# DRL-Navigation/DDRL4NAV

Measured on AMD Instinct MI355X. Metric: env-steps/sec (whole node) + PPO update ms, Pong 256 envs at 1/2/4/8 GPUs, higher is better.
Workload: dtype f32 (f16x3 MFMA planes, fp32 accumulate)

## Files before the change

ddrl4nav_amd/csrc/conv2.hip:

```cpp
#include "engine2.h"

namespace ddrl {


using bf8 = __attribute__((ext_vector_type(8))) __bf16;
using u4v = __attribute__((ext_vector_type(4))) unsigned;
using bf4 = __attribute__((ext_vector_type(4))) __bf16;

#ifndef DDRL_F1_KO
#define DDRL_F1_KO 0
#endif
#ifndef DDRL_F1_LDS_PAD
#define DDRL_F1_LDS_PAD 0
#endif
#ifndef DDRL_F1_PITCH
#define DDRL_F1_PITCH 168
#endif
template <int NE>
struct Fwd1B {
  static constexpr int ROWS = 32 * NE, A_BYTES = 4 * NPL * 2 * ROWS * 16, PITCH = DDRL_F1_PITCH, IMG_BYTES = 64 * PITCH;
  static constexpr int STAGE_BYTES = A_BYTES + IMG_BYTES, AQ = A_BYTES / 16, NAJ = AQ / 256;
  static constexpr size_t LDS_BYTES = 2 * STAGE_BYTES + DDRL_F1_LDS_PAD;
};

// ... 663 lines not shown
  {
    ProfRange pr(c.prof, acting ? "ConvFwd1.act" : "ConvFwd1", st);
    if (c.L->NE == 2) {
      launch_fwd1_planes<2>(c, acting, st);
    } else {
      launch_fwd1_planes<1>(c, acting, st);
    }
  }
  {
    ProfRange pr(c.prof, acting ? "ConvFwd2.act" : "ConvFwd2", st);
    launch_fwd2_planes(c, acting, st);
  }
  {
    ProfRange pr(c.prof, acting ? "ConvFwd3.act" : "ConvFwd3", st);
    launch_fwd3_planes(c, acting, st);
  }
}

#ifndef DDRL_D3B_THREADS
#define DDRL_D3B_THREADS 256
#endif
#ifndef DDRL_D3B_TN
#define DDRL_D3B_TN 2
#endif
struct Dgrad3B {
  static constexpr int THREADS = DDRL_D3B_THREADS, TN = DDRL_D3B_TN, SPT = ((THREADS / 64) * 32 * TN) / 81;
  static constexpr int KOC = 16, NKB = 64 / KOC, PIXB = 2 * KOC;
  static constexpr int IMG_PLANE = SPT * 121 * PIXB;
  static constexpr int W_OFF = NPL * IMG_PLANE, W_BYTES = 9 * NPL * 64 * 32;
  static constexpr int NIU = SPT * 49, NIJ = (NIU + THREADS - 1) / THREADS;
  static constexpr int NWQ = W_BYTES / 16, NWJ = (NWQ + THREADS - 1) / THREADS;
  static constexpr size_t LDS_BYTES = W_OFF + W_BYTES;
};

__global__ __launch_bounds__(Dgrad3B::THREADS) __attribute__((amdgpu_waves_per_eu(2, 2))) void conv_dgrad3_planes_kernel(
    const float* __restrict__ dz3, int64_t dz_es, const unsigned short* __restrict__ wd3b, float* __restrict__ amax, const unsigned* __restrict__ m2,
    float* __restrict__ out, int64_t out_es, int n) {
  using K = Dgrad3B;
  extern __shared__ __attribute__((aligned(16))) char ldsd3[];
  const int tid = threadIdx.x, lane = tid & 63, wc = tid >> 6, l31 = lane & 31, hi = lane >> 5;
  const int e = blockIdx.z, b0 = blockIdx.x * K::SPT;
  const float sa = plane_scale(amax[amax_idx(AMAX_DZ3, e)]), inv = 1.0f / (sa * plane_scale(amax[amax_idx(AMAX_W3, e)]));
  for (int i = tid; i < K::W_OFF / 16; i += K::THREADS) *(f4*)(ldsd3 + i * 16) = zero4();
  const float* isrc[K::NIJ];
  int idst[K::NIJ];
#pragma unroll
  for (int j = 0; j < K::NIJ; ++j) {
    const int u = min(tid + K::THREADS * j, K::NIU - 1);
    const int s = u / 49, px = u % 49;
    isrc[j] = dz3 + e * dz_es + (int64_t)min(b0 + s, n - 1) * FLAT + px;
    idst[j] = (s * 121 + (px / 7 + 2) * 11 + px % 7 + 2) * K::PIXB;
  }
  const unsigned short* wsrc = wd3b + (int64_t)e * (K::NKB * 9 * NPL * 64 * 16) + tid * 8;
  int aA[2], bB[K::TN];
#pragma unroll
  for (int i = 0; i < 2; ++i) aA[i] = K::W_OFF + (i * 32 + l31) * 32 + hi * 16;
#pragma unroll
  for (int j = 0; j < K::TN; ++j) {
    int c = wc * (32 * K::TN) + j * 32 + l31;
    if (c >= K::SPT * 81) c = 0;
    const int s = c / 81, pix = c % 81;
    bB[j] = (s * 121 + (pix / 9 + 2) * 11 + pix % 9 + 2) * K::PIXB + hi * 16;
  }
  float ir[K::NIJ][K::KOC];
  f4 wr[K::NWJ];
  auto fetch = [&](int kb) {
#pragma unroll
    for (int j = 0; j < K::NIJ; ++j)
#pragma unroll
      for (int c = 0; c < K::KOC; ++c) ir[j][c] = isrc[j][(kb * K::KOC + c) * 49];
#pragma unroll
    for (int j = 0; j < K::NWJ; ++j)
      if (j + 1 < K::NWJ || tid + K::THREADS * j < K::NWQ) wr[j] = *(const f4*)(wsrc + kb * (9 * NPL * 1024) + j * (K::THREADS * 8));
  };
  auto commit = [&]() {
#pragma unroll
    for (int j = 0; j < K::NIJ; ++j) {
      if (j + 1 < K::NIJ || tid + K::THREADS * j < K::NIU) {
        unsigned pl[K::KOC / 2][NPL];
#pragma unroll
        for (int c = 0; c < K::KOC / 2; ++c) split_planes(ir[j][2 * c], ir[j][2 * c + 1], sa, pl[c]);
        char* d = ldsd3 + idst[j];
#pragma unroll
        for (int p = 0; p < NPL; ++p) {
          *(u4v*)(d + p * K::IMG_PLANE) = (u4v){pl[0][p], pl[1][p], pl[2][p], pl[3][p]};
          *(u4v*)(d + p * K::IMG_PLANE + 16) = (u4v){pl[4][p], pl[5][p], pl[6][p], pl[7][p]};
        }
      }
    }
#pragma unroll
    for (int j = 0; j < K::NWJ; ++j)
      if (j + 1 < K::NWJ || tid + K::THREADS * j < K::NWQ) *(f4*)(ldsd3 + K::W_OFF + (tid + K::THREADS * j) * 16) = wr[j];
  };
  f32x16 acc[2][K::TN];
#pragma unroll
  for (int i = 0; i < 2; ++i)
#pragma unroll
    for (int j = 0; j < K::TN; ++j)
#pragma unroll
      for (int r = 0; r < 16; ++r) acc[i][j][r] = 0.0f;
  fetch(0);
  __syncthreads();
  commit();
  fetch(1);
  __syncthreads();
  for (int kb = 0; kb < K::NKB; ++kb) {
#pragma unroll
    for (int t = 0; t < 9; ++t) {
      constexpr int ROW11 = 11;
      const int toff = ((t / 3) * ROW11 + t % 3) * K::PIXB;
      frag8 af[NPL][2], bfr[NPL][K::TN];
#pragma unroll
      for (int p = 0; p < NPL; ++p) {
#pragma unroll
        for (int i = 0; i < 2; ++i) af[p][i] = *(const frag8*)(ldsd3 + aA[i] + (t * NPL + p) * 2048);
#pragma unroll
        for (int j = 0; j < K::TN; ++j) bfr[p][j] = *(const frag8*)(ldsd3 + bB[j] - toff + p * K::IMG_PLANE);
      }
      DDRL_PLANE_PRODUCTS;
#pragma unroll
      for (int m = 0; m < NPROD; ++m)
#pragma unroll
        for (int i = 0; i < 2; ++i)
#pragma unroll
          for (int j = 0; j < K::TN; ++j) acc[i][j] = mfma_planes(af[PA[m]][i], bfr[PB[m]][j], acc[i][j]);
    }
    __syncthreads();
    if (kb + 1 < K::NKB) {
      commit();
      if (kb + 2 < K::NKB) fetch(kb + 2);
    }
    __syncthreads();
  }
  float big = 0.0f;
#pragma unroll
  for (int j = 0; j < K::TN; ++j) {
    const int c = wc * (32 * K::TN) + j * 32 + l31;
    const int s = c / 81, pix = c % 81;
    if (c >= K::SPT * 81 || b0 + s >= n) continue;
    const int64_t off = (int64_t)(b0 + s) * 5184 + pix + hi * (4 * 81);
    float* op = out + e * out_es + off;
    const unsigned mw = m2[(e * (out_es / 5184) + b0 + s) * 162 + pix * 2 + hi];
#pragma unroll
    for (int i = 0; i < 2; ++i)
#pragma unroll
      for (int r = 0; r < 16; ++r) {
        const float g = leaky_bit(mw, 16 * i + 15 - r, acc[i][j][r] * inv);
        op[(i * 32 + acc_row(r, 0)) * 81] = g;
        big = fmaxf(big, fabsf(g));
      }
  }
  amax_update(big, amax + amax_idx(AMAX_DZ2, e));
}
static void launch_dgrad3_planes(const EncCall& c, hipStream_t st) {
  using K = Dgrad3B;
  const Workspace& w = *c.ws;
  static bool configured = false;
  if (!configured) {
    (void)hipFuncSetAttribute((const void*)conv_dgrad3_planes_kernel, hipFuncAttributeMaxDynamicSharedMemorySize, (int)K::LDS_BYTES);
    configured = true;
  }
  hipLaunchKernelGGL(conv_dgrad3_planes_kernel, dim3((unsigned)((c.n + K::SPT - 1) / K::SPT), 1, (unsigned)c.L->NE), dim3(K::THREADS), K::LDS_BYTES, st,
                     w.dz3, c.max_batch * FLAT, w.wd3b, w.amax, w.m2, w.dz2, c.max_batch * 5184, c.n);
}

void launch_conv_dgrad3_2(const EncCall& c, hipStream_t st) {
  ProfRange pr(c.prof, "ConvDgrad3", st);
  launch_dgrad3_planes(c, st);
}

#ifndef DDRL_D2_KO
#define DDRL_D2_KO 0
#endif
struct Dgrad2Both {
  static constexpr int SPT = 5, THREADS = 512, TN = 2;
  static constexpr int IMG_PLANE = SPT * 121 * 16;
  static constexpr int W_HALF = 2 * NPL * 64 * 32;
  static constexpr int W_OFF = NPL * IMG_PLANE, W_BYTES = 2 * W_HALF;
  static constexpr int NIU = SPT * 81;
  static constexpr int NWQ = W_BYTES / 16, NWJ = NWQ / THREADS;
  static constexpr size_t LDS_BYTES = W_OFF + W_BYTES;
};

__global__ __launch_bounds__(512) __attribute__((amdgpu_waves_per_eu(2, 2))) void conv_dgrad2_both_kernel(
    const float* __restrict__ dz2, int64_t dz_es, const unsigned short* __restrict__ wd2b, float* __restrict__ amax, float* __restrict__ out,
    int64_t out_es, int n) {
  using K = Dgrad2Both;
  extern __shared__ __attribute__((aligned(16))) char ldsd2[];
  const int tid = threadIdx.x, lane = tid & 63, wc = tid >> 6, l31 = lane & 31, hi = lane >> 5;
  const int e = blockIdx.y, b0 = blockIdx.x * K::SPT;
  const float sa = plane_scale(amax[amax_idx(AMAX_DZ2, e)]), inv = 1.0f / (sa * plane_scale(amax[amax_idx(AMAX_W2, e)]));
  for (int i = tid; i < K::W_OFF / 16; i += K::THREADS) *(f4*)(ldsd2 + i * 16) = zero4();
  const int u = min(tid, K::NIU - 1);
  const float* isrc = dz2 + e * dz_es + (int64_t)min(b0 + u / 81, n - 1) * 5184 + u % 81;
  const int idst = ((u / 81) * 121 + ((u % 81) / 9 + 1) * 11 + (u % 81) % 9 + 1) * 16;
  const unsigned short* wsrc[K::NWJ];
#pragma unroll
  for (int j = 0; j < K::NWJ; ++j) {
    const int q = tid + K::THREADS * j, par = q / (K::W_HALF / 16), qh = q % (K::W_HALF / 16);
    wsrc[j] = wd2b + (int64_t)(e * 2 + par) * (8 * 2 * NPL * 64 * 16) + qh * 8;
  }
  int aA[4], bB[K::TN];
#pragma unroll
  for (int i = 0; i < 4; ++i) aA[i] = K::W_OFF + (i >> 1) * K::W_HALF + ((i & 1) * 32 + l31) * 32 + hi * 16;
#pragma unroll
  for (int j = 0; j < K::TN; ++j) {
    int c = wc * (32 * K::TN) + j * 32 + l31;
    if (c >= K::SPT * 100) c = 0;
    const int s = c / 100, pq = c % 100;
    bB[j] = (s * 121 + (pq / 10 + 1) * 11 + (pq % 10 + 1) - hi) * 16;
  }
  float ir[8];
  f4 wr[K::NWJ];
  auto fetch = [&](int kb) {
#pragma unroll
    for (int c = 0; c < 8; ++c) ir[c] = isrc[(kb * 8 + c) * 81];
#pragma unroll
    for (int j = 0; j < K::NWJ; ++j) wr[j] = *(const f4*)(wsrc[j] + kb * (2 * NPL * 1024));
  };
  auto commit = [&]() {
    if (tid < K::NIU) {
      unsigned pl[4][NPL];
#pragma unroll
      for (int c = 0; c < 4; ++c) split_planes(ir[2 * c], ir[2 * c + 1], sa, pl[c]);
      char* d = ldsd2 + idst;
#pragma unroll
      for (int p = 0; p < NPL; ++p) *(u4v*)(d + p * K::IMG_PLANE) = (u4v){pl[0][p], pl[1][p], pl[2][p], pl[3][p]};
    }
#pragma unroll
    for (int j = 0; j < K::NWJ; ++j) *(f4*)(ldsd2 + K::W_OFF + (tid + K::THREADS * j) * 16) = wr[j];
  };
  f32x16 acc[4][K::TN];
#pragma unroll
  for (int i = 0; i < 4; ++i)
#pragma unroll
    for (int j = 0; j < K::TN; ++j)
#pragma unroll
      for (int r = 0; r < 16; ++r) acc[i][j][r] = 0.0f;
  constexpr int NKB = 8;
  fetch(0);
  __syncthreads();
  commit();
  fetch(1);
  __syncthreads();
  for (int kb = 0; kb < NKB; ++kb) {
#pragma unroll
    for (int kg = 0; kg < 2; ++kg) {
      frag8 af[NPL][4], bfr[NPL][K::TN];
#pragma unroll
      for (int p = 0; p < NPL; ++p) {
#pragma unroll
        for (int i = 0; i < 4; ++i) af[p][i] = *(const frag8*)(ldsd2 + aA[i] + (kg * NPL + p) * 2048);
#pragma unroll
        for (int j = 0; j < K::TN; ++j) bfr[p][j] = *(const frag8*)(ldsd2 + bB[j] + p * K::IMG_PLANE - kg * (11 * 16));
      }
      DDRL_PLANE_PRODUCTS;
#pragma unroll
      for (int t = 0; t < NPROD; ++t)
#pragma unroll
        for (int i = 0; i < 4; ++i)
#pragma unroll
          for (int j = 0; j < K::TN; ++j) acc[i][j] = mfma_planes(af[PA[t]][i], bfr[PB[t]][j], acc[i][j]);
    }
    __syncthreads();
    if (kb + 1 < NKB) {
      commit();
      if (kb + 2 < NKB) fetch(kb + 2);
    }
    __syncthreads();
  }
  float big = 0.0f;
#pragma unroll
  for (int j = 0; j < K::TN; ++j) {
    const int c = wc * (32 * K::TN) + j * 32 + l31;
    const int s = c / 100, pq = c % 100;
    if (c >= K::SPT * 100 || b0 + s >= n) continue;
#pragma unroll
    for (int a = 0; a < 2; ++a) {
      float* base = out + e * out_es + (int64_t)(b0 + s) * 12800 + (2 * (pq / 10) + a) * 20 + 2 * (pq % 10);
#pragma unroll
      for (int r = 0; r < 16; ++r) {
        const float g0 = acc[2 * a][j][r] * inv, g1 = acc[2 * a + 1][j][r] * inv;
        *(float2*)(base + acc_row(r, hi) * 400) = make_float2(g0, g1);
        big = fmaxf(big, fmaxf(fabsf(g0), fabsf(g1)));
      }
    }
  }
  amax_update(big, amax + amax_idx(AMAX_DZ1, e));
}

void launch_conv_dgrad2_2(const EncCall& c, hipStream_t st) {
  const Workspace& w = *c.ws;
  ProfRange pr(c.prof, "ConvDgrad2", st);
  static bool configured = false;
  if (!configured) {
    (void)hipFuncSetAttribute((const void*)conv_dgrad2_both_kernel, hipFuncAttributeMaxDynamicSharedMemorySize, (int)Dgrad2Both::LDS_BYTES);
    configured = true;
  }
  hipLaunchKernelGGL(conv_dgrad2_both_kernel, dim3((unsigned)((c.n + Dgrad2Both::SPT - 1) / Dgrad2Both::SPT), (unsigned)c.L->NE, 1),
                     dim3(Dgrad2Both::THREADS), Dgrad2Both::LDS_BYTES, st, w.dz2, c.max_batch * 5184, w.wd2b, w.amax, w.dz1, c.max_batch * 12800, c.n);
}

}
```

ddrl4nav_amd/csrc/fc2.hip:

```cpp
#include "engine2.h"

namespace ddrl {

using bf8f = __attribute__((ext_vector_type(8))) __bf16;

#ifndef DDRL_FC_SWZ
#define DDRL_FC_SWZ 1
#endif

struct FcFwdB {
  static constexpr int PITCH = 80, PLANE = 128 * PITCH, B_OFF = NPL * PLANE, LDS_BYTES = 2 * NPL * PLANE;
};

template <bool SPLIT>
__global__ __launch_bounds__(256) void fc_fwd_planes_kernel(const float* __restrict__ a3, int64_t a3_es, const unsigned short* __restrict__ wlb,
                                                            const float* __restrict__ amax, const float* __restrict__ params, int64_t bias_off0,
                                                            int64_t bias_off1, float* __restrict__ h, int64_t h_es, int n, int ne, int nsplit,
                                                            float* __restrict__ part, const float* __restrict__ smax, int smax_es) {
  using K = FcFwdB;
  extern __shared__ __attribute__((aligned(16))) char ldsf[];
  const int tid = threadIdx.x, lane = tid & 63, wave = tid >> 6, l31 = lane & 31, hi = lane >> 5;
  const int wr = wave >> 1, wc = wave & 1;
  int bx = blockIdx.x, by = blockIdx.y, bz = blockIdx.z;
  if (!SPLIT && DDRL_FC_SWZ != 0 && (gridDim.y & 7) == 0) {
// ... 152 lines not shown
    static bool configured = false;
    if (!configured) {
      (void)hipFuncSetAttribute((const void*)fc_fwd_planes_kernel<false>, hipFuncAttributeMaxDynamicSharedMemorySize, (int)FcFwdB::LDS_BYTES);
      (void)hipFuncSetAttribute((const void*)fc_fwd_planes_kernel<true>, hipFuncAttributeMaxDynamicSharedMemorySize, (int)FcFwdB::LDS_BYTES);
      configured = true;
    }
    const dim3 grid(FEAT / 128, (c.n + 127) / 128, c.L->NE * nsplit);
    if (nsplit > 1)
      hipLaunchKernelGGL(fc_fwd_planes_kernel<true>, grid, dim3(256), FcFwdB::LDS_BYTES, st, w.a3, MB * FLAT, w.wlb, w.amax, c.params,
                         c.L->enc_base[0] + c.L->enc.lb, c.L->enc_base[c.L->NE - 1] + c.L->enc.lb, w.h, MB * FEAT, c.n, c.L->NE, nsplit, w.wpart,
                         per_sample_max ? w.actmax : (const float*)nullptr, DDRL_ACT_FUSED_MAX);
    else
      hipLaunchKernelGGL(fc_fwd_planes_kernel<false>, grid, dim3(256), FcFwdB::LDS_BYTES, st, w.a3, MB * FLAT, w.wlb, w.amax, c.params,
                         c.L->enc_base[0] + c.L->enc.lb, c.L->enc_base[c.L->NE - 1] + c.L->enc.lb, w.h, MB * FEAT, c.n, c.L->NE, 1, w.wpart,
                         (const float*)nullptr, 0);
  }
}

#ifndef DDRL_FCD_KBK
#define DDRL_FCD_KBK 32
#endif
#ifndef DDRL_FCD_WPE
#define DDRL_FCD_WPE 2
#endif
struct FcDgradB {
  static constexpr int KBK = DDRL_FCD_KBK, WPE = DDRL_FCD_WPE, PITCH = 2 * KBK + 16, PLANE = 128 * PITCH, B_OFF = NPL * PLANE, LDS_BYTES = 2 * NPL * PLANE;
  static constexpr int NAQ = KBK / 4, ARJ = 128 * NAQ / 256, AROWS = 256 / NAQ;
  static constexpr int NWF = KBK / 8, WJ = 128 * NWF / 256, WCOLS = 256 / NWF;
};
__global__ __launch_bounds__(256) __attribute__((amdgpu_waves_per_eu(FcDgradB::WPE, FcDgradB::WPE))) void fc_dgrad_planes_kernel(const float* __restrict__ dh, int64_t dh_es, const unsigned short* __restrict__ wdlb,
                                                              float* __restrict__ amax, const unsigned* __restrict__ m3, float* __restrict__ dz3, int64_t a3_es, int n) {
  using K = FcDgradB;
  extern __shared__ __attribute__((aligned(16))) char ldsg[];
  const int tid = threadIdx.x, lane = tid & 63, wave = tid >> 6, l31 = lane & 31, hi = lane >> 5;
  const int wr = wave >> 1, wc = wave & 1;
  int bx = blockIdx.x, by = blockIdx.y;
  if (DDRL_FC_SWZ != 0 && (gridDim.y & 7) == 0) {
    const int lin = bx + 25 * by, xcd = lin & 7, q = lin >> 3;
    if ((gridDim.y & 63) != 0) {
      bx = q % 25, by = (q / 25) * 8 + xcd;
    } else {
      const int blk = q / 40, r = q % 40;
      bx = (blk % 5) * 5 + r % 5, by = ((blk / 5) * 8 + r / 5) * 8 + xcd;
    }
  }
  const int e = blockIdx.z, k0 = bx * 128, b0 = by * 128;
  const float sa = plane_scale(amax[amax_idx(AMAX_DH, e)]), inv = 1.0f / (sa * plane_scale(amax[amax_idx(AMAX_WL, e)]));
  const int n4 = tid % K::NAQ, rr = tid / K::NAQ;
  const float* asrc[K::ARJ];
#pragma unroll
  for (int j = 0; j < K::ARJ; ++j) asrc[j] = dh + e * dh_es + (int64_t)min(b0 + rr + K::AROWS * j, n - 1) * FEAT + n4 * 4;
  const int n8 = tid % K::NWF, cc = tid / K::NWF;
  const unsigned short* wsrc[K::WJ];
#pragma unroll
  for (int j = 0; j < K::WJ; ++j) wsrc[j] = wdlb + (int64_t)e * 3 * FLAT * FEAT + (int64_t)min(k0 + cc + K::WCOLS * j, FLAT - 1) * FEAT + n8 * 8;
  int aA[2], bB[2];
#pragma unroll
  for (int i = 0; i < 2; ++i) aA[i] = (wr * 64 + i * 32 + l31) * K::PITCH + hi * 16;
#pragma unroll
  for (int j = 0; j < 2; ++j) bB[j] = K::B_OFF + (wc * 64 + j * 32 + l31) * K::PITCH + hi * 16;
  f4 ar[K::ARJ], wrg[K::WJ][NPL];
  auto fetch = [&](int kb) {
#pragma unroll
    for (int j = 0; j < K::ARJ; ++j) ar[j] = ld4(asrc[j] + kb * K::KBK);
#pragma unroll
    for (int j = 0; j < K::WJ; ++j)
#pragma unroll
      for (int p = 0; p < NPL; ++p) wrg[j][p] = *(const f4*)(wsrc[j] + (int64_t)p * FLAT * FEAT + kb * K::KBK);
  };
  auto commit = [&]() {
#pragma unroll
    for (int j = 0; j < K::ARJ; ++j) {
      const f4 v = ar[j];
      unsigned pa[NPL], pb[NPL];
      split_planes_c(v.x, v.y, sa, pa);
      split_planes_c(v.z, v.w, sa, pb);
      char* d = ldsg + (rr + K::AROWS * j) * K::PITCH + n4 * 8;
#pragma unroll
      for (int p = 0; p < NPL; ++p) *(uint2*)(d + p * K::PLANE) = make_uint2(pa[p], pb[p]);
    }
#pragma unroll
    for (int j = 0; j < K::WJ; ++j)
#pragma unroll
      for (int p = 0; p < NPL; ++p) *(f4*)(ldsg + K::B_OFF + p * K::PLANE + (cc + K::WCOLS * j) * K::PITCH + n8 * 16) = wrg[j][p];
  };
  f32x16 acc[2][2];
#pragma unroll
  for (int i = 0; i < 2; ++i)
#pragma unroll
    for (int j = 0; j < 2; ++j)
#pragma unroll
      for (int r = 0; r < 16; ++r) acc[i][j][r] = 0.0f;
  constexpr int NKB = FEAT / K::KBK;
  fetch(0);
  commit();
  fetch(1);
  __syncthreads();
  for (int kb = 0; kb < NKB; ++kb) {
#pragma unroll
    for (int kg = 0; kg < K::KBK / 16; ++kg) {
      frag8 a[NPL][2], b[NPL][2];
#pragma unroll
      for (int p = 0; p < NPL; ++p) {
#pragma unroll
        for (int i = 0; i < 2; ++i) a[p][i] = *(const frag8*)(ldsg + aA[i] + p * K::PLANE + kg * 32);
#pragma unroll
        for (int j = 0; j < 2; ++j) b[p][j] = *(const frag8*)(ldsg + bB[j] + p * K::PLANE + kg * 32);
      }
      DDRL_PLANE_PRODUCTS;
#pragma unroll
      for (int t = 0; t < NPROD; ++t)
#pragma unroll
        for (int i = 0; i < 2; ++i)
#pragma unroll
          for (int j = 0; j < 2; ++j) acc[i][j] = mfma_planes(a[PA[t]][i], b[PB[t]][j], acc[i][j]);
    }
    __syncthreads();
    if (kb + 1 < NKB) {
      commit();
      if (kb + 2 < NKB) fetch(kb + 2);
    }
    __syncthreads();
  }
  float big = 0.0f;
#pragma unroll
  for (int j = 0; j < 2; ++j) {
    const int k = k0 + wc * 64 + j * 32 + l31;
    if (k >= FLAT) continue;
    const int ch = k / 49, pix = k % 49;
    const int mbit = 16 * (ch >> 5) + 15 - ((ch & 3) + 4 * ((ch & 31) >> 3));
    const unsigned* mp = m3 + (int64_t)e * (a3_es / FLAT) * 98 + pix * 2 + ((ch >> 2) & 1);
#pragma unroll
    for (int i = 0; i < 2; ++i) {
      unsigned mw[16];
#pragma unroll
      for (int r = 0; r < 16; ++r) {
        const int b = min(b0 + wr * 64 + i * 32 + acc_row(r, hi), n - 1);
        mw[r] = mp[(int64_t)b * 98];
      }
#pragma unroll
      for (int r = 0; r < 16; ++r) {
        const int b = b0 + wr * 64 + i * 32 + acc_row(r, hi);
        const float g = leaky_bit(mw[r], mbit, acc[i][j][r] * inv);
        if (b < n) {
          dz3[e * a3_es + (int64_t)b * FLAT + k] = g;
          big = fmaxf(big, fabsf(g));
        }
      }
    }
  }
  amax_update(big, amax + amax_idx(AMAX_DZ3, e));
}

using s4v = __attribute__((ext_vector_type(4))) short;
struct FcWgradB {
  static constexpr int KB = 32, PITCH = 320, PLANE = KB * PITCH, B_OFF = NPL * PLANE, LDS_BYTES = 2 * NPL * PLANE;
  static constexpr int64_t SLAB = (int64_t)FEAT * FLAT + FEAT;
};

__device__ __forceinline__ frag8 tr_fragment(const char* lds, int byte_off) {
  typedef s4v __attribute__((address_space(3))) * lds_s4;
  const s4v lo = __builtin_amdgcn_ds_read_tr16_b64_v4i16((lds_s4)(lds + byte_off));
  const s4v hi = __builtin_amdgcn_ds_read_tr16_b64_v4i16((lds_s4)(lds + byte_off + 4 * FcWgradB::PITCH));
  typedef __attribute__((ext_vector_type(8))) short s8v;
  const s8v v = __builtin_shufflevector(lo, hi, 0, 1, 2, 3, 4, 5, 6, 7);
  return __builtin_bit_cast(frag8, v);
}

__global__ __launch_bounds__(256) void fc_wgrad_planes_kernel(const float* __restrict__ dh, int64_t dh_es, const float* __restrict__ a3,
                                                              int64_t a3_es, const float* __restrict__ amax, const float* __restrict__ gsc,
                                                              int64_t gsc_es, float* __restrict__ part, int n, int nsplit, int ne) {
  using K = FcWgradB;
  extern __shared__ __attribute__((aligned(16))) char ldsw[];
  const int tid = threadIdx.x, lane = tid & 63, wave = tid >> 6, l31 = lane & 31, hi = lane >> 5;
  const int wr = wave >> 1, wc = wave & 1;
#if DDRL_FC_SWZ != 0
  const int unit = (int)(blockIdx.x >> 5) * 8 + (int)(blockIdx.x & 7);
  if (unit >= 25 * ne * nsplit) return;
  const int bx = unit % 25, by = (int)(blockIdx.x >> 3) & 3, bz = unit / 25;
#else
  const int bx = blockIdx.x, by = blockIdx.y, bz = blockIdx.z;
#endif
  const int e = bz % ne, split = bz / ne;
  const float sd = WGRAD_HEADROOM * plane_scale(amax[amax_idx(AMAX_DH, e)]) / amax[amax_idx(AMAX_GMAX, e)], sa = plane_scale(amax[amax_idx(AMAX_A3, e)]),
              inv = 1.0f / (sd * sa);
  const float* gs = gsc + e * gsc_es;
  const int k0 = bx * 128, n0 = by * 128;
  const int nkb = (n + K::KB - 1) / K::KB;
  const int per = (nkb + nsplit - 1) / nsplit;
  const int kb_begin = split * per, kb_end = min(nkb, kb_begin + per);
  const int c4 = tid & 31, kk = tid >> 5;
  const float* dsrc = dh + e * dh_es + n0 + c4 * 4;
  const float* asrc = a3 + e * a3_es + min(k0 + c4 * 4, FLAT - 4);
  const int g16 = lane >> 4, q = (lane >> 2) & 3, pp = lane & 3;
  int aA[2], bB[2];
#pragma unroll
  for (int i = 0; i < 2; ++i) aA[i] = (8 * (g16 >> 1) + q) * K::PITCH + (wr * 64 + i * 32 + 16 * (g16 & 1) + 4 * pp) * 2;
#pragma unroll
  for (int j = 0; j < 2; ++j) bB[j] = K::B_OFF + (8 * (g16 >> 1) + q) * K::PITCH + (wc * 64 + j * 32 + 16 * (g16 & 1) + 4 * pp) * 2;
  f4 dr[4], ar[4];
  float gr[4];
  f4 bsum = zero4();
  const bool bias_owner = (bx == 0);
  auto fetch = [&](int kb) {
#pragma unroll
    for (int j = 0; j < 4; ++j) {
      const int64_t row = min(kb * K::KB + kk + 8 * j, n - 1);
      dr[j] = ld4(dsrc + row * FEAT);
      ar[j] = ld4(asrc + row * FLAT);
      gr[j] = gs[row];
    }
  };
  auto commit = [&](int kb) {
    if (kb * K::KB + K::KB > n) {
      rare_path();
#pragma unroll
      for (int j = 0; j < 4; ++j)
        if (kb * K::KB + kk + 8 * j >= n) dr[j] = zero4();
      rare_path();
    }
#pragma unroll
    for (int j = 0; j < 4; ++j) {
      char* d = ldsw + (kk + 8 * j) * K::PITCH + c4 * 8;
      unsigned pa[NPL], pb[NPL];
      const float sdj = sd * gr[j];
      split_planes(dr[j].x, dr[j].y, sdj, pa);
      split_planes(dr[j].z, dr[j].w, sdj, pb);
#pragma unroll
      for (int p = 0; p < NPL; ++p) *(uint2*)(d + p * K::PLANE) = make_uint2(pa[p], pb[p]);
      split_planes(ar[j].x, ar[j].y, sa, pa);
      split_planes(ar[j].z, ar[j].w, sa, pb);
#pragma unroll
      for (int p = 0; p < NPL; ++p) *(uint2*)(d + K::B_OFF + p * K::PLANE) = make_uint2(pa[p], pb[p]);
    }
    if (bias_owner) bsum += (dr[0] * gr[0] + dr[1] * gr[1]) + (dr[2] * gr[2] + dr[3] * gr[3]);
  };
  f32x16 acc[2][2];
#pragma unroll
  for (int i = 0; i < 2; ++i)
#pragma unroll
    for (int j = 0; j < 2; ++j)
#pragma unroll
      for (int r = 0; r < 16; ++r) acc[i][j][r] = 0.0f;
  if (kb_begin < kb_end) {
    fetch(kb_begin);
    commit(kb_begin);
    if (kb_begin + 1 < kb_end) fetch(kb_begin + 1);
    __syncthreads();
    for (int kb = kb_begin; kb < kb_end; ++kb) {
#pragma unroll
      for (int kg = 0; kg < 2; ++kg) {
        frag8 a[NPL][2], b[NPL][2];
#pragma unroll
        for (int p = 0; p < NPL; ++p) {
#pragma unroll
          for (int i = 0; i < 2; ++i) a[p][i] = tr_fragment(ldsw, aA[i] + p * K::PLANE + kg * 16 * K::PITCH);
#pragma unroll
          for (int j = 0; j < 2; ++j) b[p][j] = tr_fragment(ldsw, bB[j] + p * K::PLANE + kg * 16 * K::PITCH);
        }
        DDRL_PLANE_PRODUCTS;
#pragma unroll
        for (int t = 0; t < NPROD; ++t)
#pragma unroll
          for (int i = 0; i < 2; ++i)
#pragma unroll
            for (int j = 0; j < 2; ++j) acc[i][j] = mfma_planes(a[PA[t]][i], b[PB[t]][j], acc[i][j]);
      }
      __syncthreads();
      if (kb + 1 < kb_end) {
        commit(kb + 1);
        if (kb + 2 < kb_end) fetch(kb + 2);
      }
      __syncthreads();
    }
  }
  float* slab = part + ((int64_t)split * 2 + e) * K::SLAB;
#pragma unroll
  for (int j = 0; j < 2; ++j) {
    const int k = k0 + wc * 64 + j * 32 + l31;
    if (k >= FLAT) continue;
#pragma unroll
    for (int i = 0; i < 2; ++i)
#pragma unroll
      for (int r = 0; r < 16; ++r) slab[(int64_t)(n0 + wr * 64 + i * 32 + acc_row(r, hi)) * FLAT + k] = acc[i][j][r] * inv;
  }
  if (bias_owner) {
    float* red = (float*)ldsw;
    st4(red + kk * 128 + c4 * 4, bsum);
    __syncthreads();
    if (tid < 128) {
      float s = 0.0f;
#pragma unroll
      for (int t = 0; t < 8; ++t) s += red[t * 128 + tid];
      slab[(int64_t)FEAT * FLAT + n0 + tid] = s;
    }
  }
}

void launch_fc_backward2(const EncCall& c, float* grads, hipStream_t st, int part) {
  const Workspace& w = *c.ws;
  const int64_t MB = c.max_batch;
  const ParamLayout& L = *c.L;
  const int S = c.splits->fc;
  if (part != 1) {
    {
      ProfRange pr(c.prof, "FcWgrad", st);
      static bool configured_w = false;
      if (!configured_w) {
        (void)hipFuncSetAttribute((const void*)fc_wgrad_planes_kernel, hipFuncAttributeMaxDynamicSharedMemorySize, (int)FcWgradB::LDS_BYTES);
        configured_w = true;
      }
#if DDRL_FC_SWZ != 0
      const dim3 wgrid((unsigned)((25 * L.NE * S + 7) / 8 * 32));
#else
      const dim3 wgrid((FLAT + 127) / 128, FEAT / 128, L.NE * S);
#endif
      hipLaunchKernelGGL(fc_wgrad_planes_kernel, wgrid, dim3(256), FcWgradB::LDS_BYTES, st, w.dh, MB * FEAT, w.a3, MB * FLAT, w.amax, w.gsc, MB,
                         w.wpart, c.n, S, L.NE);
    }
    ProfRange pr(c.prof, "reduce_partials", st);
    launch_reduce_partials(w.wpart, S, FcWgradB::SLAB, L.NE, grads, L.enc_base[0] + L.enc.lw, L.enc_base[1] + L.enc.lw, st);
  }
  if (part != 2) {
    ProfRange pr(c.prof, "FcDgrad", st);
    static bool configured = false;
    if (!configured) {
      (void)hipFuncSetAttribute((const void*)fc_dgrad_planes_kernel, hipFuncAttributeMaxDynamicSharedMemorySize, (int)FcDgradB::LDS_BYTES);
      configured = true;
    }
    hipLaunchKernelGGL(fc_dgrad_planes_kernel, dim3((FLAT + 127) / 128, (c.n + 127) / 128, L.NE), dim3(256), FcDgradB::LDS_BYTES, st, w.dh, MB * FEAT,
                       w.wdlb, w.amax, w.m3, w.dz3, MB * FLAT, c.n);
  }
}

}
```

Measured before the change: 252,600.

## Add row-class dgrad3 kernel that skips padded output columns

```diff
diff --git a/ddrl4nav_amd/csrc/conv2.hip b/ddrl4nav_amd/csrc/conv2.hip
--- a/ddrl4nav_amd/csrc/conv2.hip
+++ b/ddrl4nav_amd/csrc/conv2.hip
@@ -839,16 +839,176 @@
   }
   amax_update(big, amax + amax_idx(AMAX_DZ2, e));
 }
+
+#ifndef DDRL_D3_ROWS
+#define DDRL_D3_ROWS 1
+#endif
+__device__ __forceinline__ bool d3_rows_pixel(int col, int& s, int& y, int& x) {
+  const int f = col >> 5, l = col & 31;
+  if (f < 6) {
+    const int idx = min(col, 188), rem = idx % 63;
+    s = idx / 63;
+    y = 1 + rem / 9;
+    x = rem % 9;
+    return col < 189;
+  }
+  const int li = min(l, 26);
+  s = li / 9;
+  y = f == 6 ? 0 : 8;
+  x = li % 9;
+  return l < 27;
+}
+
+__global__ __launch_bounds__(256) __attribute__((amdgpu_waves_per_eu(2, 2))) void conv_dgrad3_planes_rows_kernel(
+    const float* __restrict__ dz3, int64_t dz_es, const unsigned short* __restrict__ wd3b, float* __restrict__ amax, const unsigned* __restrict__ m2,
+    float* __restrict__ out, int64_t out_es, int n) {
+  using K = Dgrad3B;
+  static_assert(K::THREADS == 256 && K::TN == 2 && K::SPT == 3, "row classes are laid out for four waves and three samples");
+  extern __shared__ __attribute__((aligned(16))) char ldsd3r[];
+  const int tid = threadIdx.x, lane = tid & 63, l31 = lane & 31, hi = lane >> 5;
+  const int wc = __builtin_amdgcn_readfirstlane(tid >> 6);
+  const int e = blockIdx.z, b0 = blockIdx.x * K::SPT;
+  const float sa = plane_scale(amax[amax_idx(AMAX_DZ3, e)]), inv = 1.0f / (sa * plane_scale(amax[amax_idx(AMAX_W3, e)]));
+  for (int i = tid; i < K::W_OFF / 16; i += K::THREADS) *(f4*)(ldsd3r + i * 16) = zero4();
+  const float* isrc[K::NIJ];
+  int idst[K::NIJ];
+#pragma unroll
+  for (int j = 0; j < K::NIJ; ++j) {
+    const int u = min(tid + K::THREADS * j, K::NIU - 1);
+    const int s = u / 49, px = u % 49;
+    isrc[j] = dz3 + e * dz_es + (int64_t)min(b0 + s, n - 1) * FLAT + px;
+    idst[j] = (s * 121 + (px / 7 + 2) * 11 + px % 7 + 2) * K::PIXB;
+  }
+  const unsigned short* wsrc = wd3b + (int64_t)e * (K::NKB * 9 * NPL * 64 * 16) + tid * 8;
+  const int X = wc & 1, grp = wc >> 1, lky = 2 * grp;
+  const int fr[3] = {3 * grp + 2 * X, 3 * grp + 1, 6 + grp};
+  const int aX = K::W_OFF + (X * 32 + l31) * 32 + hi * 16, aY = K::W_OFF + ((1 - X) * 32 + l31) * 32 + hi * 16;
+  int bB[3];
+#pragma unroll
+  for (int j = 0; j < 3; ++j) {
+    int s, y, x;
+    (void)d3_rows_pixel(fr[j] * 32 + l31, s, y, x);
+    bB[j] = (s * 121 + (y + 2) * 11 + x + 2) * K::PIXB + hi * 16;
+  }
+  const int aXl = aX + 3 * lky * NPL * 2048, bLl = bB[2] - lky * 11 * K::PIXB;
+  float ir[K::NIJ][K::KOC];
+  f4 wr[K::NWJ];
+  auto fetch = [&](int kb) {
+#pragma unroll
+    for (int j = 0; j < K::NIJ; ++j)
+#pragma unroll
+      for (int c = 0; c < K::KOC; ++c) ir[j][c] = isrc[j][(kb * K::KOC + c) * 49];
+#pragma unroll
+    for (int j = 0; j < K::NWJ; ++j)
+      if (j + 1 < K::NWJ || tid + K::THREADS * j < K::NWQ) wr[j] = *(const f4*)(wsrc + kb * (9 * NPL * 1024) + j * (K::THREADS * 8));
+  };
+  auto commit = [&]() {
+#pragma unroll
+    for (int j = 0; j < K::NIJ; ++j) {
+      if (j + 1 < K::NIJ || tid + K::THREADS * j < K::NIU) {
+        unsigned pl[K::KOC / 2][NPL];
+#pragma unroll
+        for (int c = 0; c < K::KOC / 2; ++c) split_planes(ir[j][2 * c], ir[j][2 * c + 1], sa, pl[c]);
+        char* d = ldsd3r + idst[j];
+#pragma unroll
+        for (int p = 0; p < NPL; ++p) {
+          *(u4v*)(d + p * K::IMG_PLANE) = (u4v){pl[0][p], pl[1][p], pl[2][p], pl[3][p]};
+          *(u4v*)(d + p * K::IMG_PLANE + 16) = (u4v){pl[4][p], pl[5][p], pl[6][p], pl[7][p]};
+        }
+      }
+    }
+#pragma unroll
+    for (int j = 0; j < K::NWJ; ++j)
+      if (j + 1 < K::NWJ || tid + K::THREADS * j < K::NWQ) *(f4*)(ldsd3r + K::W_OFF + (tid + K::THREADS * j) * 16) = wr[j];
+  };
+  f32x16 acc[4];
+#pragma unroll
+  for (int u = 0; u < 4; ++u)
+#pragma unroll
+    for (int r = 0; r < 16; ++r) acc[u][r] = 0.0f;
+  fetch(0);
+  __syncthreads();
+  commit();
+  fetch(1);
+  __syncthreads();
+  for (int kb = 0; kb < K::NKB; ++kb) {
+    DDRL_PLANE_PRODUCTS;
+#pragma unroll
+    for (int t = 0; t < 9; ++t) {
+      const int toff = ((t / 3) * 11 + t % 3) * K::PIXB;
+      frag8 ax[NPL], ay[NPL], ba[NPL], bb[NPL];
+#pragma unroll
+      for (int p = 0; p < NPL; ++p) {
+        ax[p] = *(const frag8*)(ldsd3r + aX + (t * NPL + p) * 2048);
+        ay[p] = *(const frag8*)(ldsd3r + aY + (t * NPL + p) * 2048);
+        ba[p] = *(const frag8*)(ldsd3r + bB[0] - toff + p * K::IMG_PLANE);
+        bb[p] = *(const frag8*)(ldsd3r + bB[1] - toff + p * K::IMG_PLANE);
+      }
+#pragma unroll
+      for (int m = 0; m < NPROD; ++m) {
+        acc[0] = mfma_planes(ax[PA[m]], ba[PB[m]], acc[0]);
+        acc[1] = mfma_planes(ay[PA[m]], ba[PB[m]], acc[1]);
+        acc[2] = mfma_planes(ax[PA[m]], bb[PB[m]], acc[2]);
+      }
+    }
+#pragma unroll
+    for (int kx = 0; kx < 3; ++kx) {
+      frag8 ax[NPL], bl[NPL];
+#pragma unroll
+      for (int p = 0; p < NPL; ++p) {
+        ax[p] = *(const frag8*)(ldsd3r + aXl + (kx * NPL + p) * 2048);
+        bl[p] = *(const frag8*)(ldsd3r + bLl - kx * K::PIXB + p * K::IMG_PLANE);
+      }
+#pragma unroll
+      for (int m = 0; m < NPROD; ++m) acc[3] = mfma_planes(ax[PA[m]], bl[PB[m]], acc[3]);
+    }
+    __syncthreads();
+    if (kb + 1 < K::NKB) {
+      commit();
+      if (kb + 2 < K::NKB) fetch(kb + 2);
+    }
+    __syncthreads();
+  }
+  float big = 0.0f;
+#pragma unroll
+  for (int u = 0; u < 4; ++u) {
+    const int i = (u == 1) ? 1 - X : X, f = fr[u == 0 || u == 1 ? 0 : (u == 2 ? 1 : 2)];
+    int s, y, x;
+    if (!d3_rows_pixel(f * 32 + l31, s, y, x) || b0 + s >= n) continue;
+    const int pix = y * 9 + x;
+    float* op = out + e * out_es + (int64_t)(b0 + s) * 5184 + pix + hi * (4 * 81);
+    const unsigned mw = m2[(e * (out_es / 5184) + b0 + s) * 162 + pix * 2 + hi];
+#pragma unroll
+    for (int r = 0; r < 16; ++r) {
+      const float g = leaky_bit(mw, 16 * i + 15 - r, acc[u][r] * inv);
+      op[(i * 32 + acc_row(r, 0)) * 81] = g;
+      big = fmaxf(big, fabsf(g));
+    }
+  }
+  amax_update(big, amax + amax_idx(AMAX_DZ2, e));
+}
+
 static void launch_dgrad3_planes(const EncCall& c, hipStream_t st) {
   using K = Dgrad3B;
   const Workspace& w = *c.ws;
+  const dim3 grid((unsigned)((c.n + K::SPT - 1) / K::SPT), 1, (unsigned)c.L->NE);
+#if DDRL_D3_ROWS
+  static bool configured_r = false;
+  if (!configured_r) {
+    (void)hipFuncSetAttribute((const void*)conv_dgrad3_planes_rows_kernel, hipFuncAttributeMaxDynamicSharedMemorySize, (int)K::LDS_BYTES);
+    configured_r = true;
+  }
+  hipLaunchKernelGGL(conv_dgrad3_planes_rows_kernel, grid, dim3(K::THREADS), K::LDS_BYTES, st, w.dz3, c.max_batch * FLAT, w.wd3b, w.amax, w.m2, w.dz2,
+                     c.max_batch * 5184, c.n);
+#else
   static bool configured = false;
   if (!configured) {
     (void)hipFuncSetAttribute((const void*)conv_dgrad3_planes_kernel, hipFuncAttributeMaxDynamicSharedMemorySize, (int)K::LDS_BYTES);
     configured = true;
   }
-  hipLaunchKernelGGL(conv_dgrad3_planes_kernel, dim3((unsigned)((c.n + K::SPT - 1) / K::SPT), 1, (unsigned)c.L->NE), dim3(K::THREADS), K::LDS_BYTES, st,
-                     w.dz3, c.max_batch * FLAT, w.wd3b, w.amax, w.m2, w.dz2, c.max_batch * 5184, c.n);
+  hipLaunchKernelGGL(conv_dgrad3_planes_kernel, grid, dim3(K::THREADS), K::LDS_BYTES, st, w.dz3, c.max_batch * FLAT, w.wd3b, w.amax, w.m2, w.dz2,
+                     c.max_batch * 5184, c.n);
+#endif
 }
 
 void launch_conv_dgrad3_2(const EncCall& c, hipStream_t st) {
```

Result: no change. 254,100 (median of 6 runs) (+0.6%).

## Double-buffer LDS stages in FC weight-gradient kernel to drop a barrier

Applied to the files above, without the earlier changes.

```diff
diff --git a/ddrl4nav_amd/csrc/fc2.hip b/ddrl4nav_amd/csrc/fc2.hip
--- a/ddrl4nav_amd/csrc/fc2.hip
+++ b/ddrl4nav_amd/csrc/fc2.hip
@@ -328,9 +328,13 @@
   amax_update(big, amax + amax_idx(AMAX_DZ3, e));
 }
 
+#ifndef DDRL_FCW_STAGES
+#define DDRL_FCW_STAGES 2
+#endif
 using s4v = __attribute__((ext_vector_type(4))) short;
 struct FcWgradB {
-  static constexpr int KB = 32, PITCH = 320, PLANE = KB * PITCH, B_OFF = NPL * PLANE, LDS_BYTES = 2 * NPL * PLANE;
+  static constexpr int KB = 32, PITCH = 320, PLANE = KB * PITCH, B_OFF = NPL * PLANE, STAGE = 2 * NPL * PLANE, STAGES = DDRL_FCW_STAGES,
+                       LDS_BYTES = STAGES * STAGE;
   static constexpr int64_t SLAB = (int64_t)FEAT * FLAT + FEAT;
 };
 
@@ -387,7 +391,7 @@
       gr[j] = gs[row];
     }
   };
-  auto commit = [&](int kb) {
+  auto commit = [&](int kb, char* stage) {
     if (kb * K::KB + K::KB > n) {
       rare_path();
 #pragma unroll
@@ -397,7 +401,7 @@
     }
 #pragma unroll
     for (int j = 0; j < 4; ++j) {
-      char* d = ldsw + (kk + 8 * j) * K::PITCH + c4 * 8;
+      char* d = stage + (kk + 8 * j) * K::PITCH + c4 * 8;
       unsigned pa[NPL], pb[NPL];
       const float sdj = sd * gr[j];
       split_planes(dr[j].x, dr[j].y, sdj, pa);
@@ -418,36 +422,51 @@
     for (int j = 0; j < 2; ++j)
 #pragma unroll
       for (int r = 0; r < 16; ++r) acc[i][j][r] = 0.0f;
+  auto compute = [&](const char* stage) {
+#pragma unroll
+    for (int kg = 0; kg < 2; ++kg) {
+      frag8 a[NPL][2], b[NPL][2];
+#pragma unroll
+      for (int p = 0; p < NPL; ++p) {
+#pragma unroll
+        for (int i = 0; i < 2; ++i) a[p][i] = tr_fragment(stage, aA[i] + p * K::PLANE + kg * 16 * K::PITCH);
+#pragma unroll
+        for (int j = 0; j < 2; ++j) b[p][j] = tr_fragment(stage, bB[j] + p * K::PLANE + kg * 16 * K::PITCH);
+      }
+      DDRL_PLANE_PRODUCTS;
+#pragma unroll
+      for (int t = 0; t < NPROD; ++t)
+#pragma unroll
+        for (int i = 0; i < 2; ++i)
+#pragma unroll
+          for (int j = 0; j < 2; ++j) acc[i][j] = mfma_planes(a[PA[t]][i], b[PB[t]][j], acc[i][j]);
+    }
+  };
   if (kb_begin < kb_end) {
     fetch(kb_begin);
-    commit(kb_begin);
+    commit(kb_begin, ldsw);
     if (kb_begin + 1 < kb_end) fetch(kb_begin + 1);
     __syncthreads();
-    for (int kb = kb_begin; kb < kb_end; ++kb) {
-#pragma unroll
-      for (int kg = 0; kg < 2; ++kg) {
-        frag8 a[NPL][2], b[NPL][2];
-#pragma unroll
-        for (int p = 0; p < NPL; ++p) {
-#pragma unroll
-          for (int i = 0; i < 2; ++i) a[p][i] = tr_fragment(ldsw, aA[i] + p * K::PLANE + kg * 16 * K::PITCH);
-#pragma unroll
-          for (int j = 0; j < 2; ++j) b[p][j] = tr_fragment(ldsw, bB[j] + p * K::PLANE + kg * 16 * K::PITCH);
+    if constexpr (K::STAGES == 2) {
+      for (int kb = kb_begin; kb < kb_end; ++kb) {
+        const int i = kb - kb_begin;
+        if (kb + 1 < kb_end) {
+          commit(kb + 1, ldsw + ((i + 1) & 1) * K::STAGE);
+          if (kb + 2 < kb_end) fetch(kb + 2);
         }
-        DDRL_PLANE_PRODUCTS;
-#pragma unroll
-        for (int t = 0; t < NPROD; ++t)
-#pragma unroll
-          for (int i = 0; i < 2; ++i)
-#pragma unroll
-            for (int j = 0; j < 2; ++j) acc[i][j] = mfma_planes(a[PA[t]][i], b[PB[t]][j], acc[i][j]);
-      }
-      __syncthreads();
-      if (kb + 1 < kb_end) {
-        commit(kb + 1);
-        if (kb + 2 < kb_end) fetch(kb + 2);
-      }
-      __syncthreads();
+        compute(ldsw + (i & 1) * K::STAGE);
+        __syncthreads();
+      }
+    } else {
+      for (int kb = kb_begin; kb < kb_end; ++kb) {
+        compute(ldsw);
+        __syncthreads();
+        if (kb + 1 < kb_end) {
+          commit(kb + 1, ldsw);
+          if (kb + 2 < kb_end) fetch(kb + 2);
+        }
+        __syncthreads();
+      }
     }
   }
   float* slab = part + ((int64_t)split * 2 + e) * K::SLAB;
```

After: 246,900 before, 247,900 after (median of 6 runs). No clear change (+0.4%).

## Add persistent double-buffered pipelined kernels for conv dgrad3 and dgrad2

Applied to the files above, without the earlier changes.

```diff
diff --git a/ddrl4nav_amd/csrc/conv2.hip b/ddrl4nav_amd/csrc/conv2.hip
--- a/ddrl4nav_amd/csrc/conv2.hip
+++ b/ddrl4nav_amd/csrc/conv2.hip
@@ -839,9 +839,161 @@
   }
   amax_update(big, amax + amax_idx(AMAX_DZ2, e));
 }
+
+static int device_cus() {
+  static int cus = 0;
+  if (cus == 0) {
+    int dev = 0;
+    (void)hipGetDevice(&dev);
+    if (hipDeviceGetAttribute(&cus, hipDeviceAttributeMultiprocessorCount, dev) != hipSuccess || cus <= 0) cus = 256;
+  }
+  return cus;
+}
+
+#ifndef DDRL_D3_PIPE
+#ifdef DDRL_PLANES_BF16
+#define DDRL_D3_PIPE 0
+#else
+#define DDRL_D3_PIPE 1
+#endif
+#endif
+#ifndef DDRL_D3_PIN
+#define DDRL_D3_PIN 2
+#endif
+struct Dgrad3P {
+  static constexpr int THREADS = 512, SPT = 3, NCOL = SPT * 81;
+  static constexpr int KOC = 16, NKB = 64 / KOC, PIXB = 2 * KOC;
+  static constexpr int IMG_PLANE = SPT * 121 * PIXB;
+  static constexpr int W_OFF = NPL * IMG_PLANE, W_BYTES = 9 * NPL * 64 * 32, STAGE = W_OFF + W_BYTES;
+  static constexpr int NIU = SPT * 49, NHU = 2 * NIU;
+  static constexpr int NWQ = W_BYTES / 16, NWJ = (NWQ + THREADS - 1) / THREADS;
+  static constexpr size_t LDS_BYTES = 2 * (size_t)STAGE;
+  static_assert(NCOL <= (THREADS / 64) * 32 && NHU <= THREADS && NKB % 2 == 0, "one fragment tile per wave, one half-unit per thread");
+  static_assert(!DDRL_D3_PIPE || (STAGE % 16 == 0 && LDS_BYTES <= 160 * 1024), "LDS budget");
+};
+
+__global__ __launch_bounds__(512) void conv_dgrad3_pipe_kernel(const float* __restrict__ dz3, int64_t dz_es, const unsigned short* __restrict__ wd3b,
+                                                                float* __restrict__ amax, const unsigned* __restrict__ m2, float* __restrict__ out,
+                                                                int64_t out_es, int n) {
+  using K = Dgrad3P;
+  extern __shared__ __attribute__((aligned(16))) char ldsd3p[];
+  const int tid = threadIdx.x, lane = tid & 63, wc = tid >> 6, l31 = lane & 31, hi = lane >> 5;
+  const int e = blockIdx.y, ntiles = (n + K::SPT - 1) / K::SPT, G = gridDim.x;
+  const float sa = plane_scale(amax[amax_idx(AMAX_DZ3, e)]), inv = 1.0f / (sa * plane_scale(amax[amax_idx(AMAX_W3, e)]));
+  for (int i = tid; i < (int)(K::LDS_BYTES / 16); i += K::THREADS) *(f4*)(ldsd3p + i * 16) = zero4();
+  const int hu = min(tid, K::NHU - 1), half = hu / K::NIU, u = hu % K::NIU, us = u / 49, px = u % 49;
+  const float* isrc = dz3 + e * dz_es + half * (8 * 49) + px;
+  const int idst = (us * 121 + (px / 7 + 2) * 11 + px % 7 + 2) * K::PIXB + half * 16;
+  const unsigned short* wsrc[K::NWJ];
+#pragma unroll
+  for (int j = 0; j < K::NWJ; ++j) wsrc[j] = wd3b + (int64_t)e * (K::NKB * 9 * NPL * 64 * 16) + min(tid + K::THREADS * j, K::NWQ - 1) * 8;
+  int aA[2];
+#pragma unroll
+  for (int i = 0; i < 2; ++i) aA[i] = K::W_OFF + (i * 32 + l31) * 32 + hi * 16;
+  int col = wc * 32 + l31;
+  if (col >= K::NCOL) col = 0;
+  const int bB = ((col / 81) * 121 + ((col % 81) / 9 + 2) * 11 + (col % 81) % 9 + 2) * K::PIXB + hi * 16;
+  float ir[8];
+  f4 wr[K::NWJ];
+  auto fetch = [&](int tile, int kb) __attribute__((always_inline)) {
+    const float* src = isrc + (int64_t)min(tile * K::SPT + us, n - 1) * FLAT + kb * (K::KOC * 49);
+#pragma unroll
+    for (int c = 0; c < 8; ++c) ir[c] = src[c * 49];
+#pragma unroll
+    for (int j = 0; j < K::NWJ; ++j) wr[j] = *(const f4*)(wsrc[j] + kb * (9 * NPL * 1024));
+  };
+  auto commit = [&](int stage) __attribute__((always_inline)) {
+    char* sb = ldsd3p + stage * K::STAGE;
+    unsigned pl[4][NPL];
+#pragma unroll
+    for (int c = 0; c < 4; ++c) split_planes(ir[2 * c], ir[2 * c + 1], sa, pl[c]);
+#pragma unroll
+    for (int p = 0; p < NPL; ++p) *(u4v*)(sb + idst + p * K::IMG_PLANE) = (u4v){pl[0][p], pl[1][p], pl[2][p], pl[3][p]};
+#pragma unroll
+    for (int j = 0; j < K::NWJ; ++j) *(f4*)(sb + K::W_OFF + min(tid + K::THREADS * j, K::NWQ - 1) * 16) = wr[j];
+  };
+  const int c = wc * 32 + l31, s = c / 81, pix = c % 81;
+  const unsigned* msrc = m2 + (int64_t)e * (out_es / 5184) * 162 + pix * 2 + hi;
+  int tile = blockIdx.x;
+  fetch(tile, 0);
+  __syncthreads();
+  commit(0);
+  fetch(tile, 1);
+  __syncthreads();
+  float big = 0.0f;
+  for (; tile < ntiles; tile += G) {
+    const int tn = tile + G, b0 = tile * K::SPT;
+    unsigned mw = msrc[min(b0 + s, n - 1) * 162];
+    f32x16 acc[2];
+#pragma unroll
+    for (int i = 0; i < 2; ++i)
+#pragma unroll
+      for (int r = 0; r < 16; ++r) acc[i][r] = 0.0f;
+#pragma unroll
+    for (int kb = 0; kb < K::NKB; ++kb) {
+      const char* sb = ldsd3p + (kb & 1) * K::STAGE;
+#pragma unroll
+      for (int t = 0; t < 9; ++t) {
+        constexpr int ROW11 = 11;
+        const int toff = ((t / 3) * ROW11 + t % 3) * K::PIXB;
+        frag8 af[NPL][2], bfr[NPL];
+#pragma unroll
+        for (int p = 0; p < NPL; ++p) {
+#pragma unroll
+          for (int i = 0; i < 2; ++i) af[p][i] = *(const frag8*)(sb + aA[i] + (t * NPL + p) * 2048);
+          bfr[p] = *(const frag8*)(sb + bB - toff + p * K::IMG_PLANE);
+        }
+        DDRL_PLANE_PRODUCTS;
+#pragma unroll
+        for (int m = 0; m < NPROD; ++m)
+#pragma unroll
+          for (int i = 0; i < 2; ++i) acc[i] = mfma_planes(af[PA[m]][i], bfr[PB[m]], acc[i]);
+        if (t == 0) commit((kb + 1) & 1);
+        if (t == 1) fetch(kb + 2 < K::NKB ? tile : tn, (kb + 2) % K::NKB);
+#if DDRL_D3_PIN
+        __builtin_amdgcn_sched_group_barrier(0x100, 3 * NPL, 0);
+#pragma unroll
+        for (int k = 0; k < 2 * NPROD; ++k) {
+          __builtin_amdgcn_sched_group_barrier(0x008, 1, 0);
+          __builtin_amdgcn_sched_group_barrier(0x020, 3, 0);
+          __builtin_amdgcn_sched_group_barrier(0x002, DDRL_D3_PIN, 0);
+        }
+        __builtin_amdgcn_sched_group_barrier(0x200, NPL + K::NWJ, 0);
+        __builtin_amdgcn_sched_barrier(0);
+#endif
+      }
+      __syncthreads();
+      if (kb == 0) asm volatile("" : "+v"(mw));
+    }
+    if (c < K::NCOL && b0 + s < n) {
+      float* op = out + e * out_es + (int64_t)(b0 + s) * 5184 + pix + hi * (4 * 81);
+#pragma unroll
+      for (int i = 0; i < 2; ++i)
+#pragma unroll
+        for (int r = 0; r < 16; ++r) {
+          const float g = leaky_bit(mw, 16 * i + 15 - r, acc[i][r] * inv);
+          op[(i * 32 + acc_row(r, 0)) * 81] = g;
+          big = fmaxf(big, fabsf(g));
+        }
+    }
+  }
+  amax_update(big, amax + amax_idx(AMAX_DZ2, e));
+}
+
 static void launch_dgrad3_planes(const EncCall& c, hipStream_t st) {
+  const Workspace& w = *c.ws;
+#if DDRL_D3_PIPE
+  using K = Dgrad3P;
+  static bool configured = false;
+  if (!configured) {
+    (void)hipFuncSetAttribute((const void*)conv_dgrad3_pipe_kernel, hipFuncAttributeMaxDynamicSharedMemorySize, (int)K::LDS_BYTES);
+    configured = true;
+  }
+  const unsigned tiles = (unsigned)((c.n + K::SPT - 1) / K::SPT), per_enc = (unsigned)std::max(1, device_cus() / c.L->NE);
+  hipLaunchKernelGGL(conv_dgrad3_pipe_kernel, dim3(std::min(tiles, per_enc), (unsigned)c.L->NE, 1), dim3(K::THREADS), K::LDS_BYTES, st, w.dz3,
+                     c.max_batch * FLAT, w.wd3b, w.amax, w.m2, w.dz2, c.max_batch * 5184, c.n);
+#else
   using K = Dgrad3B;
-  const Workspace& w = *c.ws;
   static bool configured = false;
   if (!configured) {
     (void)hipFuncSetAttribute((const void*)conv_dgrad3_planes_kernel, hipFuncAttributeMaxDynamicSharedMemorySize, (int)K::LDS_BYTES);
@@ -849,6 +1001,7 @@
   }
   hipLaunchKernelGGL(conv_dgrad3_planes_kernel, dim3((unsigned)((c.n + K::SPT - 1) / K::SPT), 1, (unsigned)c.L->NE), dim3(K::THREADS), K::LDS_BYTES, st,
                      w.dz3, c.max_batch * FLAT, w.wd3b, w.amax, w.m2, w.dz2, c.max_batch * 5184, c.n);
+#endif
 }
 
 void launch_conv_dgrad3_2(const EncCall& c, hipStream_t st) {
@@ -976,16 +1129,161 @@
   amax_update(big, amax + amax_idx(AMAX_DZ1, e));
 }
 
+#ifndef DDRL_D2_PIPE
+#define DDRL_D2_PIPE 1
+#endif
+#ifndef DDRL_D2_PIN
+#define DDRL_D2_PIN 2
+#endif
+struct Dgrad2Pipe : Dgrad2Both {
+  static constexpr int STAGE = (int)Dgrad2Both::LDS_BYTES;
+  static constexpr size_t LDS_BYTES = 2 * (size_t)STAGE;
+  static_assert(STAGE % 16 == 0 && LDS_BYTES <= 160 * 1024, "LDS budget");
+};
+
+__global__ __launch_bounds__(512) __attribute__((amdgpu_waves_per_eu(2, 2))) void conv_dgrad2_pipe_kernel(
+    const float* __restrict__ dz2, int64_t dz_es, const unsigned short* __restrict__ wd2b, float* __restrict__ amax, float* __restrict__ out,
+    int64_t out_es, int n) {
+  using K = Dgrad2Pipe;
+  extern __shared__ __attribute__((aligned(16))) char ldsd2p[];
+  const int tid = threadIdx.x, lane = tid & 63, wc = tid >> 6, l31 = lane & 31, hi = lane >> 5;
+  const int e = blockIdx.y, ntiles = (n + K::SPT - 1) / K::SPT, G = gridDim.x;
+  const float sa = plane_scale(amax[amax_idx(AMAX_DZ2, e)]), inv = 1.0f / (sa * plane_scale(amax[amax_idx(AMAX_W2, e)]));
+  for (int i = tid; i < (int)(K::LDS_BYTES / 16); i += K::THREADS) *(f4*)(ldsd2p + i * 16) = zero4();
+  const int u = min(tid, K::NIU - 1), us = u / 81;
+  const float* isrc = dz2 + e * dz_es + u % 81;
+  const int idst = (us * 121 + ((u % 81) / 9 + 1) * 11 + (u % 81) % 9 + 1) * 16;
+  const unsigned short* wsrc[K::NWJ];
+#pragma unroll
+  for (int j = 0; j < K::NWJ; ++j) {
+    const int q = tid + K::THREADS * j, par = q / (K::W_HALF / 16), qh = q % (K::W_HALF / 16);
+    wsrc[j] = wd2b + (int64_t)(e * 2 + par) * (8 * 2 * NPL * 64 * 16) + qh * 8;
+  }
+  int aA[4], bB[K::TN];
+#pragma unroll
+  for (int i = 0; i < 4; ++i) aA[i] = K::W_OFF + (i >> 1) * K::W_HALF + ((i & 1) * 32 + l31) * 32 + hi * 16;
+#pragma unroll
+  for (int j = 0; j < K::TN; ++j) {
+    int c = wc * (32 * K::TN) + j * 32 + l31;
+    if (c >= K::SPT * 100) c = 0;
+    const int s = c / 100, pq = c % 100;
+    bB[j] = (s * 121 + (pq / 10 + 1) * 11 + (pq % 10 + 1) - hi) * 16;
+  }
+  float ir[8];
+  f4 wr[K::NWJ];
+  auto fetch = [&](int tile, int kb) __attribute__((always_inline)) {
+    const float* src = isrc + (int64_t)min(tile * K::SPT + us, n - 1) * 5184 + kb * (8 * 81);
+#pragma unroll
+    for (int c = 0; c < 8; ++c) ir[c] = src[c * 81];
+#pragma unroll
+    for (int j = 0; j < K::NWJ; ++j) wr[j] = *(const f4*)(wsrc[j] + kb * (2 * NPL * 1024));
+  };
+  auto commit = [&](int stage) __attribute__((always_inline)) {
+    char* sb = ldsd2p + stage * K::STAGE;
+    unsigned pl[4][NPL];
+#pragma unroll
+    for (int c = 0; c < 4; ++c) split_planes(ir[2 * c], ir[2 * c + 1], sa, pl[c]);
+#pragma unroll
+    for (int p = 0; p < NPL; ++p) *(u4v*)(sb + idst + p * K::IMG_PLANE) = (u4v){pl[0][p], pl[1][p], pl[2][p], pl[3][p]};
+#pragma unroll
+    for (int j = 0; j < K::NWJ; ++j) *(f4*)(sb + K::W_OFF + (tid + K::THREADS * j) * 16) = wr[j];
+  };
+  constexpr int NKB = 8;
+  int tile = blockIdx.x;
+  fetch(tile, 0);
+  __syncthreads();
+  commit(0);
+  fetch(tile, 1);
+  __syncthreads();
+  float big = 0.0f;
+  for (; tile < ntiles; tile += G) {
+    const int tn = tile + G;
+    f32x16 acc[4][K::TN];
+#pragma unroll
+    for (int i = 0; i < 4; ++i)
+#pragma unroll
+      for (int j = 0; j < K::TN; ++j)
+#pragma unroll
+        for (int r = 0; r < 16; ++r) acc[i][j][r] = 0.0f;
+#pragma unroll
+    for (int kb = 0; kb < NKB; ++kb) {
+      const char* sb = ldsd2p + (kb & 1) * K::STAGE;
+#pragma unroll
+      for (int kg = 0; kg < 2; ++kg) {
+        frag8 af[NPL][4], bfr[NPL][K::TN];
+#pragma unroll
+        for (int p = 0; p < NPL; ++p) {
+#pragma unroll
+          for (int i = 0; i < 4; ++i) af[p][i] = *(const frag8*)(sb + aA[i] + (kg * NPL + p) * 2048);
+#pragma unroll
+          for (int j = 0; j < K::TN; ++j) bfr[p][j] = *(const frag8*)(sb + bB[j] + p * K::IMG_PLANE - kg * (11 * 16));
+        }
+        DDRL_PLANE_PRODUCTS;
+#pragma unroll
+        for (int t = 0; t < NPROD; ++t)
+#pragma unroll
+          for (int i = 0; i < 4; ++i)
+#pragma unroll
+            for (int j = 0; j < K::TN; ++j) acc[i][j] = mfma_planes(af[PA[t]][i], bfr[PB[t]][j], acc[i][j]);
+        if (kg == 0) commit((kb + 1) & 1);
+        else fetch(kb + 2 < NKB ? tile : tn, (kb + 2) % NKB);
+#if DDRL_D2_PIN
+        __builtin_amdgcn_sched_group_barrier(0x100, NPL * (4 + K::TN), 0);
+#pragma unroll
+        for (int k = 0; k < NPROD * 4 * K::TN; ++k) {
+          __builtin_amdgcn_sched_group_barrier(0x008, 1, 0);
+          __builtin_amdgcn_sched_group_barrier(0x020, 1, 0);
+          __builtin_amdgcn_sched_group_barrier(0x002, DDRL_D2_PIN, 0);
+        }
+        __builtin_amdgcn_sched_group_barrier(0x200, NPL + K::NWJ, 0);
+        __builtin_amdgcn_sched_barrier(0);
+#endif
+      }
+      __syncthreads();
+    }
+    const int b0 = tile * K::SPT;
+#pragma unroll
+    for (int j = 0; j < K::TN; ++j) {
+      const int c = wc * (32 * K::TN) + j * 32 + l31;
+      const int s = c / 100, pq = c % 100;
+      if (c >= K::SPT * 100 || b0 + s >= n) continue;
+#pragma unroll
+      for (int a = 0; a < 2; ++a) {
+        float* base = out + e * out_es + (int64_t)(b0 + s) * 12800 + (2 * (pq / 10) + a) * 20 + 2 * (pq % 10);
+#pragma unroll
+        for (int r = 0; r < 16; ++r) {
+          const float g0 = acc[2 * a][j][r] * inv, g1 = acc[2 * a + 1][j][r] * inv;
+          *(float2*)(base + acc_row(r, hi) * 400) = make_float2(g0, g1);
+          big = fmaxf(big, fmaxf(fabsf(g0), fabsf(g1)));
+        }
+      }
+    }
+  }
+  amax_update(big, amax + amax_idx(AMAX_DZ1, e));
+}
+
 void launch_conv_dgrad2_2(const EncCall& c, hipStream_t st) {
   const Workspace& w = *c.ws;
   ProfRange pr(c.prof, "ConvDgrad2", st);
+  const unsigned tiles = (unsigned)((c.n + Dgrad2Both::SPT - 1) / Dgrad2Both::SPT);
+#if DDRL_D2_PIPE
+  static bool configured = false;
+  if (!configured) {
+    (void)hipFuncSetAttribute((const void*)conv_dgrad2_pipe_kernel, hipFuncAttributeMaxDynamicSharedMemorySize, (int)Dgrad2Pipe::LDS_BYTES);
+    configured = true;
+  }
+  const unsigned per_enc = (unsigned)std::max(1, device_cus() / c.L->NE);
+  hipLaunchKernelGGL(conv_dgrad2_pipe_kernel, dim3(std::min(tiles, per_enc), (unsigned)c.L->NE, 1), dim3(Dgrad2Pipe::THREADS), Dgrad2Pipe::LDS_BYTES, st,
+                     w.dz2, c.max_batch * 5184, w.wd2b, w.amax, w.dz1, c.max_batch * 12800, c.n);
+#else
   static bool configured = false;
   if (!configured) {
     (void)hipFuncSetAttribute((const void*)conv_dgrad2_both_kernel, hipFuncAttributeMaxDynamicSharedMemorySize, (int)Dgrad2Both::LDS_BYTES);
     configured = true;
   }
-  hipLaunchKernelGGL(conv_dgrad2_both_kernel, dim3((unsigned)((c.n + Dgrad2Both::SPT - 1) / Dgrad2Both::SPT), (unsigned)c.L->NE, 1),
-                     dim3(Dgrad2Both::THREADS), Dgrad2Both::LDS_BYTES, st, w.dz2, c.max_batch * 5184, w.wd2b, w.amax, w.dz1, c.max_batch * 12800, c.n);
-}
-
-}
+  hipLaunchKernelGGL(conv_dgrad2_both_kernel, dim3(tiles, (unsigned)c.L->NE, 1), dim3(Dgrad2Both::THREADS), Dgrad2Both::LDS_BYTES, st, w.dz2,
+                     c.max_batch * 5184, w.wd2b, w.amax, w.dz1, c.max_batch * 12800, c.n);
+#endif
+}
+
+}
```

Measured after the change: 260,500 before, 262,500 after, median of 6. Within noise of the previous version (+0.8%).
